# peach-xiao/EMRT

Measured on AMD Instinct MI355X. Metric: training tiles/sec at 256x256, higher is better.
Workload: dtype bf16; 1 GPU; EMRT ResNet50, Potsdam 256x256, 6 classes, batch 8 per GPU, fwd+bwd+SGD step (BASELINE configs[1]), bf16; global_batch=8, parallelism=dp1, hipgraph=True

## Files before the change

### emrt_amd/csrc/common.hpp

```cpp
#pragma once
#include <hip/hip_runtime.h>
#include <stdint.h>
#include <stdio.h>
#include <string.h>
#include "../../include/emrt_hip.h"

#define EMRT_F32 0
#define EMRT_BF16 1
#define EMRT_F16 2

namespace emrt {

extern thread_local char g_err[512];
inline int fail(const char* fn, const char* msg) {
  snprintf(g_err, sizeof(g_err), "%s: %s", fn, msg);
  return -1;
}
inline int check_launch(const char* fn) {
  hipError_t e = hipGetLastError();
  if (e != hipSuccess) {
    snprintf(g_err, sizeof(g_err), "%s: launch failed: %s", fn, hipGetErrorString(e));
    return -2;
  }
  return 0;
}
#define EMRT_REQUIRE(cond, msg) \
  do {                          \
    if (!(cond)) return emrt::fail(__func__, msg); \
  } while (0)

struct Tuning {
  int conv_tile;
  int wgrad_split;
  int thin_cblk;
  int thin_blocks;
  int thin_ch;
  int no_thin_bwd;
  int igemm64_nst;
  int wgrad_nst;
  int pair_max;
  int msda_fwd_global;
  int msda_bwd_global;
  int msda_lds_min_pairs;
  int msda_bwd_dref_lds;
  int msda_band_halo;
  int msda_scatter_qsplit;
  int msda_scatter_cuts;
  int msda_fwd_chunks;
  int msda_fwd_threads;
  int msda_fwd_probe;
  int bn_block_kb;
  int bn_slice_c;
  int bn_operand_blocks;
  int ln_bwd_rows;
  int ln_bwd_max_blocks;
  int ln_bwd_threads;
  int ln_atomic;
  int gn_group_blocks;
  int gn_stat_rows;
  int gn_bwd_stat_rows;
  int gn_apply_rows;
  int igemm8p_probe;
  int igemm8p_cmajor;
  int igemm8p_min_blocks;
  int wgrad8p_min_steps;
  int wgrad8p_slab;
  int wgrad8p_xcd;
  int wgrad8p_force;
  int no_ksplit128;
  int wgrad_no_overwrite;
  int no_s2_dgrad;
  int wgroup_blocks;
  int wgroup_min_steps;
  int wgroup_max;
  int wgroup8;
  int wgroup8_blocks;
  int wgroup8_min_work;
  int msda_scatter_merge;
  int msda_scatter_mfma;
  int msda_mf_bands;
  int sgd_nt;
  int mha_bwd_split;
  int mha_valu;
  int no_bna;
  int memcpy_kernel;
  int xk;
};
extern Tuning g_tune;

struct Scratch {
  void* ptr; size_t bytes; void* stream;
  unsigned* tick;
  float* xk_part;
};
constexpr size_t SCRATCH_TICK_BYTES = 65536;
constexpr int SCRATCH_TICKS = (int)(SCRATCH_TICK_BYTES / 4);
constexpr size_t SCRATCH_XK_BYTES = 8u << 20;
extern Scratch g_scratch;

struct bf16_t {
  unsigned short v;
};
struct f16_t {
  unsigned short v;
};

__device__ __forceinline__ float to_f32(float x) { return x; }
__device__ __forceinline__ float to_f32(bf16_t x) { return __uint_as_float(((uint32_t)x.v) << 16); }
__device__ __forceinline__ float to_f32(f16_t x) { return (float)__builtin_bit_cast(_Float16, x.v); }
__device__ __forceinline__ float bf16_bits_to_f32(uint32_t lo16) { return __uint_as_float(lo16 << 16); }
__device__ __forceinline__ float f16_bits_to_f32(uint32_t lo16) { return (float)__builtin_bit_cast(_Float16, (unsigned short)lo16); }

template <class T>
__device__ __forceinline__ T from_f32(float f);
template <>
__device__ __forceinline__ float from_f32<float>(float f) {
  return f;
}
template <>
__device__ __forceinline__ bf16_t from_f32<bf16_t>(float f) {
  __bf16 b = (__bf16)f;
  bf16_t r;
  r.v = __builtin_bit_cast(unsigned short, b);
  return r;
}
template <>
__device__ __forceinline__ f16_t from_f32<f16_t>(float f) {
  f16_t r;
  r.v = __builtin_bit_cast(unsigned short, (_Float16)f);
  return r;
}
typedef __attribute__((ext_vector_type(2))) _Float16 emrt_half2_t;
typedef __attribute__((ext_vector_type(2))) float emrt_float2_t;
__device__ __forceinline__ uint32_t pack_f16x2(float lo, float hi) {
  emrt_half2_t h = __builtin_convertvector((emrt_float2_t){lo, hi}, emrt_half2_t);
  return __builtin_bit_cast(uint32_t, h);
}
__device__ __forceinline__ void unpack_f16x2(uint32_t w, float& lo, float& hi) {
  const emrt_half2_t h = __builtin_bit_cast(emrt_half2_t, w);
  lo = (float)h.x;
  hi = (float)h.y;
}
__device__ __forceinline__ uint32_t pack_bf16x2(float lo, float hi) {
  return (uint32_t)from_f32<bf16_t>(lo).v | ((uint32_t)from_f32<bf16_t>(hi).v << 16);
}

template <class T>
struct Vec4;
template <>
struct Vec4<float> {
  __device__ static __forceinline__ void load(const float* p, float (&o)[4]) {
    float4 v = *reinterpret_cast<const float4*>(p);
    o[0] = v.x; o[1] = v.y; o[2] = v.z; o[3] = v.w;
  }
  __device__ static __forceinline__ void store(float* p, const float (&o)[4]) {
    *reinterpret_cast<float4*>(p) = make_float4(o[0], o[1], o[2], o[3]);
  }
// ... 230 lines not shown
```

### emrt_amd/csrc/conv.hip

```cpp
#include "common.hpp"
#include "bn_operand.hpp"
#include <stdlib.h>
#include <type_traits>

using namespace emrt;

typedef __attribute__((ext_vector_type(8))) __bf16 bf16x8_t;
typedef __attribute__((ext_vector_type(4))) short short4_t;
typedef __attribute__((ext_vector_type(16))) float f32x16_t;

struct ConvArgs {
  const void* in = nullptr;
  const void* w = nullptr;
  void* out = nullptr;
  const float* bias = nullptr;
  const float* scale = nullptr;
  const void* res = nullptr;
  int N = 0, H = 0, W = 0, C = 0, ldin = 0;
  long long in_bs = 0;
  int OH = 0, OW = 0, OC = 0, ldout = 0;
  long long out_bs = 0;
  int ldres = 0;
  long long res_bs = 0;
  int KH = 0, KW = 0, stride = 0, pad = 0;
  int dil = 1;
  int relu = 0, out_f32 = 0;
  int cmajor = 0;
  double* stats = nullptr;
  const void* mask_y = nullptr;
  float mask_scale = 1.f;
  const void* stat_x = nullptr;
  int ldsx = 0;
  long long sx_bs = 0;
  int ldy = 0;
  long long y_bs = 0;
  int xk_S = 0;
  float* xk_part = nullptr;
  unsigned* xk_tick = nullptr;
  const unsigned long long* drop_seed = nullptr;
  unsigned drop_salt = 0;
  float drop_p = 0.f;
  BnOperand bna = {};
  void* a_out = nullptr;
};

template <class T>
__device__ __forceinline__ void mma_chunk(f32x16_t& acc, const uint4& a, const uint4& b);
template <>
__device__ __forceinline__ void mma_chunk<bf16_t>(f32x16_t& acc, const uint4& a, const uint4& b) {
  acc = __builtin_amdgcn_mfma_f32_32x32x16_bf16(__builtin_bit_cast(bf16x8_t, a), __builtin_bit_cast(bf16x8_t, b), acc, 0, 0, 0);
}
typedef __attribute__((ext_vector_type(8))) _Float16 f16x8_t;
template <>
__device__ __forceinline__ void mma_chunk<f16_t>(f32x16_t& acc, const uint4& a, const uint4& b) {
  acc = __builtin_amdgcn_mfma_f32_32x32x16_f16(__builtin_bit_cast(f16x8_t, a), __builtin_bit_cast(f16x8_t, b), acc, 0, 0, 0);
}
template <>
__device__ __forceinline__ void mma_chunk<float>(f32x16_t& acc, const uint4& a, const uint4& b) {
  acc = __builtin_amdgcn_mfma_f32_32x32x2f32(__uint_as_float(a.x), __uint_as_float(b.x), acc, 0, 0, 0);
  acc = __builtin_amdgcn_mfma_f32_32x32x2f32(__uint_as_float(a.y), __uint_as_float(b.y), acc, 0, 0, 0);
  acc = __builtin_amdgcn_mfma_f32_32x32x2f32(__uint_as_float(a.z), __uint_as_float(b.z), acc, 0, 0, 0);
  acc = __builtin_amdgcn_mfma_f32_32x32x2f32(__uint_as_float(a.w), __uint_as_float(b.w), acc, 0, 0, 0);
}

constexpr unsigned BUF_RANGE = 0x80000000u;
constexpr unsigned BUF_OOB = 0x80000000u;
typedef __attribute__((ext_vector_type(4))) unsigned int u32x4_t;
__device__ __forceinline__ uint4 buf_load16(__amdgpu_buffer_rsrc_t rs, unsigned off) {
  const u32x4_t v = __builtin_amdgcn_raw_buffer_load_b128(rs, (int)off, 0, 0);
  return make_uint4(v.x, v.y, v.z, v.w);
}
template <class T>
__device__ __forceinline__ uint32_t buf_load_elem(__amdgpu_buffer_rsrc_t rs, unsigned off);
template <>
__device__ __forceinline__ uint32_t buf_load_elem<bf16_t>(__amdgpu_buffer_rsrc_t rs, unsigned off) {
  return (uint32_t)(unsigned short)__builtin_amdgcn_raw_buffer_load_b16(rs, (int)off, 0, 0);
}
template <>
__device__ __forceinline__ uint32_t buf_load_elem<f16_t>(__amdgpu_buffer_rsrc_t rs, unsigned off) {
  return (uint32_t)(unsigned short)__builtin_amdgcn_raw_buffer_load_b16(rs, (int)off, 0, 0);
}
template <>
__device__ __forceinline__ uint32_t buf_load_elem<float>(__amdgpu_buffer_rsrc_t rs, unsigned off) {
  return (uint32_t)__builtin_amdgcn_raw_buffer_load_b32(rs, (int)off, 0, 0);
// ... 1281 lines not shown
  if (G > 1 && lds < (size_t)(G - 1) * 16 * 256 * 4) lds = (size_t)(G - 1) * 16 * 256 * 4;
  static bool attr_done = false;
  if (!attr_done) {
    if (hipFuncSetAttribute(reinterpret_cast<const void*>(igemm_bna_kernel<T, 2>), hipFuncAttributeMaxDynamicSharedMemorySize, 160 * 1024) != hipSuccess ||
        hipFuncSetAttribute(reinterpret_cast<const void*>(igemm_bna_kernel<T, 4>), hipFuncAttributeMaxDynamicSharedMemorySize, 160 * 1024) != hipSuccess)
      return fail("emrt_conv2d_bna", "cannot raise the dynamic LDS limit");
    attr_done = true;
  }
  if (G == 1) hipLaunchKernelGGL((igemm_bna_kernel<T, 1>), dim3((unsigned)nb), dim3(256), lds, st, a);
  else if (G == 2) hipLaunchKernelGGL((igemm_bna_kernel<T, 2>), dim3((unsigned)nb), dim3(512), lds, st, a);
  else hipLaunchKernelGGL((igemm_bna_kernel<T, 4>), dim3((unsigned)nb), dim3(1024), lds, st, a);
  return check_launch("emrt_conv2d_bna");
}

static ConvArgs bna_args(const void* in, const void* w_packed, void* out, const float* bias, const void* residual, int N, int H, int W, int C, int ldin,
                         long long in_bs, int OH, int OW, int OC, int ldout, long long out_bs, int ldres, long long res_bs, int KH, int KW, int stride, int pad,
                         int relu, int out_f32, double* bn_stats, int dilation, const double* sums, double count, float eps, float momentum, float* mean,
                         float* invstd, float* run_mean, float* run_var, const float* gamma, const float* beta, int in_relu, void* a_out) {
  ConvArgs a = conv_fwd_args(in, w_packed, out, bias, residual, N, H, W, C, ldin, in_bs, OH, OW, OC, ldout, out_bs, ldres, res_bs, KH, KW, stride, pad, dilation,
                             relu, out_f32, bn_stats, 0, nullptr);
  a.bna.sums = sums; a.bna.inv_count = count > 0.0 ? 1.0 / count : 0.0; a.bna.eps = eps; a.bna.momentum = momentum; a.bna.mean = mean; a.bna.invstd = invstd;
  a.bna.run_mean = run_mean; a.bna.run_var = run_var; a.bna.gamma = gamma; a.bna.beta = beta; a.bna.relu = in_relu;
  a.a_out = a_out;
  return a;
}

extern "C" int emrt_conv2d_bna_supported(const void* in, const void* w_packed, void* out, const float* bias, const void* residual, int N, int H, int W, int C,
                                         int ldin, long long in_bs, int OH, int OW, int OC, int ldout, long long out_bs, int ldres, long long res_bs, int KH,
                                         int KW, int stride, int pad, int relu, int out_f32, double* bn_stats, int dilation, const double* sums, double count,
                                         float eps, float momentum, float* mean, float* invstd, float* run_mean, float* run_var, const float* gamma,
                                         const float* beta, int in_relu, void* a_out, int dtype, void* stream) {
  if (!(dtype == EMRT_F32 || dtype == EMRT_BF16) || !in || !w_packed || !out || !sums || !mean || !invstd || !gamma || !beta || !a_out || count <= 0.0) return 0;
  if (N <= 0 || H <= 0 || W <= 0 || C <= 0 || OC <= 0 || dilation < 1 || g_tune.no_bna == 1) return 0;
  const long long esz = dtype == EMRT_F32 ? 4 : 2;
  if ((long long)N * H * W * C * esz >= (1ll << 31) || (long long)N * H * W + 512 >= (1ll << 31)) return 0;
  if (((long long)(N - 1) * in_bs + ((long long)H * W - 1) * ldin + C) * esz >= (1ll << 31) || (long long)OC * KH * KW * C * esz >= (1ll << 31)) return 0;
  const ConvArgs a = bna_args(in, w_packed, out, bias, residual, N, H, W, C, ldin, in_bs, OH, OW, OC, ldout, out_bs, ldres, res_bs, KH, KW, stride, pad, relu, out_f32,
                              bn_stats, dilation, sums, count, eps, momentum, mean, invstd, run_mean, run_var, gamma, beta, in_relu, a_out);
  hipStream_t st = (hipStream_t)stream;
  return with_train_dtype("emrt_conv2d_bna_supported", dtype, [&](auto t) { return bna_plan<decltype(t)>(a, st).kind != CONV_NONE ? 1 : 0; });
}

extern "C" int emrt_conv2d_bna(const void* in, const void* w_packed, void* out, const float* bias, const void* residual, int N, int H, int W, int C,
                               int ldin, long long in_bs, int OH, int OW, int OC, int ldout, long long out_bs, int ldres, long long res_bs, int KH,
                               int KW, int stride, int pad, int relu, int out_f32, double* bn_stats, int dilation, const double* sums, double count,
                               float eps, float momentum, float* mean, float* invstd, float* run_mean, float* run_var, const float* gamma,
                               const float* beta, int in_relu, void* a_out, int dtype, void* stream) {
  EMRT_REQUIRE_TRAIN_DTYPE(dtype);
  EMRT_REQUIRE(in && w_packed && out && sums && mean && invstd && gamma && beta && a_out, "null pointer");
  const ConvShape s = {N, H, W, C, OH, OW, OC, KH, KW, stride, pad, dilation};
  EMRT_CONV_CHECK(s, 0, 0, 0, 0, dtype, CK_DIMS);
  EMRT_REQUIRE(dilation >= 1 && count > 0.0, "bad dims");
  EMRT_REQUIRE((run_mean != nullptr) == (run_var != nullptr), "running statistics come in pairs");
  EMRT_REQUIRE(a_out != out && a_out != in, "a_out is a buffer of its own");
  EMRT_REQUIRE((long long)N * OH * OW + 512 < (1ll << 31), "more than 2^31 pixels (32-bit pixel arithmetic)");
  EMRT_CONV_CHECK(s, ldin, in_bs, 0, 0, dtype, CK_X | CK_W);
  EMRT_REQUIRE((long long)N * H * W * C * (dtype == EMRT_F32 ? 4 : 2) < (1ll << 31), "operand spans 2 GiB or more (32-bit buffer offsets)");
  const ConvArgs a = bna_args(in, w_packed, out, bias, residual, N, H, W, C, ldin, in_bs, OH, OW, OC, ldout, out_bs, ldres, res_bs, KH, KW, stride, pad, relu, out_f32,
                              bn_stats, dilation, sums, count, eps, momentum, mean, invstd, run_mean, run_var, gamma, beta, in_relu, a_out);
  hipStream_t st = (hipStream_t)stream;
  return with_train_dtype("emrt_conv2d_bna", dtype, [&](auto t) {
    using T = decltype(t);
    const ConvPlan plan = bna_plan<T>(a, st);
    if (plan.kind == CONV_NONE) return fail("emrt_conv2d_bna", "this layer has no operand-transform kernel (ask emrt_conv2d_bna_supported first)");
    return launch_bna<T>(a, st, plan);
  });
}

template <class T>
static bool wgrad_is_vec(const WgradArgs& a) {
  constexpr int EPC = 16 / (int)sizeof(T);
  return (a.C % EPC == 0) && (a.OC % EPC == 0) && (a.ldx % EPC == 0) && (a.lddy % EPC == 0) && (a.x_bs % EPC == 0) && (a.dy_bs % EPC == 0) &&
         (((uintptr_t)a.x) % 16 == 0) && (((uintptr_t)a.dy) % 16 == 0);
}

template <class T>
static void wgrad_plan(WgradArgs& a, int& tx, int& ty, int& S_out) {
  using Cfg = WgradCfg<T>;
  const int K = a.KH * a.KW * a.C;
  const long long M = (long long)a.N * a.OH * a.OW;
  tx = (K + 127) / 128;
  ty = (a.OC + 127) / 128;
  const long long mt_total = (M + Cfg::BKM - 1) / Cfg::BKM;
  const double atom_us = (double)tx * 128.0 * (double)ty * 128.0 * 4.0 / 1.3e6;
  long long S = 1;
  double best = 1e30;
  static const int cand[] = {1, 2, 4, 8, 16, 32, 64, 128};
  for (int ci = 0; ci < (int)(sizeof(cand) / sizeof(cand[0])); ++ci) {
    const long long sc = cand[ci];
    if (sc > mt_total) break;
    if (sc > 1 && (long long)tx * ty >= 256) break;
    const double per = (double)((mt_total + sc - 1) / sc);
    const double nblk = (double)tx * ty * sc;
    const double t = per * (nblk > 1024.0 ? nblk / 1024.0 : 1.0) + sc * atom_us;
    if (t < best) { best = t; S = sc; }
  }
  if (g_tune.wgrad_split > 0) S = g_tune.wgrad_split < mt_total ? g_tune.wgrad_split : mt_total;
  a.tiles_per_split = (int)((mt_total + S - 1) / S);
  S_out = (int)((mt_total + a.tiles_per_split - 1) / a.tiles_per_split);
}

#include "wgrad8p.hpp"

template <class T>
static int wgrad_dispatch(const WgradArgs& a0, hipStream_t st) {
  using Cfg = WgradCfg<T>;
  WgradArgs a = a0;
  if constexpr (std::is_same<T, bf16_t>::value) {
    int tk, toc, S8, per;
    if (wgrad8p_plan<T>(a, tk, toc, S8, per)) return launch_wgrad8p(a, tk, toc, S8, per, st);
  }
  const bool vec = wgrad_is_vec<T>(a);
  int tx, ty, S;
  wgrad_plan<T>(a, tx, ty, S);
  if (S > 1 || !vec || g_tune.wgrad_no_overwrite) a.overwrite = 0;
  constexpr int G = 1;
  const int gv = vec ? G : 1;
  const size_t lds = (size_t)gv * 2 * 2 * Cfg::BKM * Cfg::PITCH;
  static bool attr_done = false;
  if (!attr_done) {
    if (hipFuncSetAttribute(reinterpret_cast<const void*>(wgrad_kernel<T, true, G>), hipFuncAttributeMaxDynamicSharedMemorySize,
                            (int)((size_t)G * 4 * Cfg::BKM * Cfg::PITCH)) != hipSuccess ||
        hipFuncSetAttribute(reinterpret_cast<const void*>(wgrad_kernel<T, false, 1>), hipFuncAttributeMaxDynamicSharedMemorySize,
                            (int)((size_t)4 * Cfg::BKM * Cfg::PITCH)) != hipSuccess)
      return fail("emrt_conv2d_wgrad", "cannot raise the dynamic LDS limit");
    attr_done = true;
  }
  const int xcd = g_tune.wgrad8p_xcd;
  const unsigned grid1 = 8u * (unsigned)(((long long)tx * ty * S + 7) / 8);
  if (vec && g_tune.wgrad_nst == 3) {
    static bool attr3 = false;
    if (!attr3) { (void)hipFuncSetAttribute(reinterpret_cast<const void*>(wgrad_kernel<T, true, G, 3>), hipFuncAttributeMaxDynamicSharedMemorySize, (int)((size_t)G * 4 * Cfg::BKM * Cfg::PITCH)); attr3 = true; }
    hipLaunchKernelGGL((wgrad_kernel<T, true, G, 3>), dim3(grid1), dim3(256 * G), lds, st, a, tx, ty, S, xcd);
  } else if (vec) hipLaunchKernelGGL((wgrad_kernel<T, true, G>), dim3(grid1), dim3(256 * G), lds, st, a, tx, ty, S, xcd);
  else hipLaunchKernelGGL((wgrad_kernel<T, false, 1>), dim3(grid1), dim3(256), lds, st, a, tx, ty, S, xcd);
  return check_launch("emrt_conv2d_wgrad");
}

extern "C" int emrt_conv2d_wgrad(const void* x, const void* dy, float* dw,
                                 int N, int H, int W, int C, int ldx, long long x_bs,
                                 int OH, int OW, int OC, int lddy, long long dy_bs,
                                 int KH, int KW, int stride, int pad, float* dbias, int dilation, int dtype, void* stream) {
  EMRT_REQUIRE(x && dy && dw, "null pointer");
  const ConvShape s = {N, H, W, C, OH, OW, OC, KH, KW, stride, pad, dilation};
  EMRT_CONV_CHECK(s, ldx, x_bs, lddy, dy_bs, dtype, CK_DIMS);
  EMRT_REQUIRE(dilation >= 1, "bad dims");
  EMRT_CONV_CHECK(s, ldx, x_bs, lddy, dy_bs, dtype, CK_SIZE | CK_PIXELS);
  EMRT_REQUIRE_TRAIN_DTYPE(dtype);
  EMRT_CONV_CHECK(s, ldx, x_bs, lddy, dy_bs, dtype, CK_X | CK_Y | CK_X24);
  const WgradArgs a = wgrad_args(x, dy, dw, dbias, N, H, W, C, ldx, x_bs, OH, OW, OC, lddy, dy_bs, KH, KW, stride, pad, dilation, 0);
  hipStream_t st = (hipStream_t)stream;
  return with_train_dtype("emrt_conv2d_wgrad", dtype, [&](auto t) { return wgrad_dispatch<decltype(t)>(a, st); });
}

struct ThinBwdArgs {
  const void* x; const void* dy; const void* wd; void* dx; float* dw; float* dbias; double* stats; const void* mask_y;
  int HW, C, OC, ldx, lddy, lddx, ldy, accumulate, pix_per_block, cg_shift;
  float mask_scale;
  long long x_bs, dy_bs, dx_bs, y_bs, M;
  const float* bn_mean; const float* bn_invstd; const float* bn_gamma; const float* bn_beta;
};

template <class T, int CH>
struct VecN;
template <class T>
struct VecN<T, 4> : Vec4<T> {};
template <class T>
struct VecN<T, 8> : Vec8<T> {};

template <class T, int CH, int MASK, bool ACC, bool BNX = false>
__global__ __launch_bounds__(256, CH == 4 ? 4 : 2) void thin_bwd_kernel(ThinBwdArgs p) {
  constexpr int U = 2;
  using V = VecN<T, CH>;
  __shared__ float red[32 * 256];
  const T* x = (const T*)p.x;
  const T* dy = (const T*)p.dy;
  const T* wd = (const T*)p.wd;
  const T* ym = (const T*)p.mask_y;
  T* dx = (T*)p.dx;
// ... 519 lines not shown
    w = wgrad_args(b.x, b.dy, b.dw, b.dbias, b.N, b.H, b.W, b.C, b.ldx, b.x_bs, b.OH, b.OW, b.OC, b.lddy, b.dy_bs, b.KH, b.KW, b.stride, b.pad, 1, 0);
    const bool vec = conv_is_vec<T>(d) && wgrad_is_vec<T>(w) && d.OC > 32;
    groupable = groupable && vec;
    int tx = 1, ty = 1, S = 1;
    if (vec) wgrad_plan<T>(w, tx, ty, S);
    g.nd[i] = (int)conv_blocks(d, 64, 64);
    g.wtx[i] = tx; g.wty[i] = ty;
    g.first[i] = (int)total;
    total += g.nd[i] + (long long)tx * ty * S;
  }
  for (int i = n; i <= EMRT_MAX_GROUP; ++i) g.first[i] = (int)total;
  for (int i = n; i < EMRT_MAX_GROUP; ++i) { g.d[i] = g.d[0]; g.w[i] = g.w[0]; g.nd[i] = 0; g.wtx[i] = 1; g.wty[i] = 1; }
  if (!groupable || total > 4096) {
    for (int i = 0; i < n; ++i) {
      const int rc = conv_bwd_dispatch<T>(g.d[i], g.w[i], st);
      if (rc) return rc;
    }
    return 0;
  }
  auto kern = bwd_group_kernel<T>;
  const size_t lds_d = (size_t)2 * 128 * 144, lds_w = (size_t)4 * Cfg::BKM * Cfg::PITCH;
  const size_t lds = lds_d > lds_w ? lds_d : lds_w;
  static bool attr_done = false;
  if (!attr_done) {
    if (hipFuncSetAttribute(reinterpret_cast<const void*>(kern), hipFuncAttributeMaxDynamicSharedMemorySize, (int)lds) != hipSuccess)
      return fail("emrt_conv2d_bwd_group", "cannot raise the dynamic LDS limit");
    attr_done = true;
  }
  hipLaunchKernelGGL(kern, dim3((unsigned)total), dim3(256), lds, st, g);
  return check_launch("emrt_conv2d_bwd_group");
}

extern "C" int emrt_conv2d_bwd_group(const EmrtConvBwdDesc* descs, int n, int dtype, void* stream) {
  EMRT_REQUIRE(descs && n >= 1 && n <= EMRT_MAX_GROUP, "1..6 problems");
  EMRT_REQUIRE_TRAIN_DTYPE(dtype);
  for (int i = 0; i < n; ++i) {
    const EmrtConvBwdDesc& b = descs[i];
    EMRT_REQUIRE(b.x && b.dy && b.w_bwd_packed && b.dx, "null pointer");
    EMRT_REQUIRE((b.dw == nullptr) == (descs[0].dw == nullptr) && (b.dw || !b.dbias), "dw == NULL (data gradients only) must hold for every problem of the group, without dbias");
    const ConvShape s = {b.N, b.H, b.W, b.C, b.OH, b.OW, b.OC, b.KH, b.KW, b.stride, b.pad, 1};
    EMRT_CONV_CHECK(s, b.ldx, b.x_bs, b.lddy, b.dy_bs, dtype, CK_GROUPED | CK_DIMS | CK_SIZE | CK_PIXELS);
    EMRT_REQUIRE(b.lddx >= b.C && b.dx_bs >= 0, "bad dx strides");
    EMRT_CONV_CHECK(s, b.ldx, b.x_bs, b.lddy, b.dy_bs, dtype, CK_GROUPED | CK_X | CK_Y | CK_X24);
  }
  hipStream_t st = (hipStream_t)stream;
  return with_train_dtype("emrt_conv2d_bwd_group", dtype, [&](auto t) { return conv_bwd_group_dispatch<decltype(t)>(descs, n, st); });
}

template <class T>
static int conv_dgrad_multi_dispatch(const EmrtConvDgradDesc* descs, int n, hipStream_t st) {
  ConvGroupArgs g;
  for (int i = 0; i < n; ++i) {
    const EmrtConvDgradDesc& b = descs[i];
    g.p[i] = conv_dgrad_args(b.dy, b.w_bwd_packed, b.dx, b.lddx, b.dx_bs, b.accumulate, b.addend, b.ldadd, b.add_bs, b.N, b.H, b.W, b.C, b.OH, b.OW, b.OC, b.lddy,
                             b.dy_bs, b.KH, b.KW, b.stride, b.pad, b.dilation, g_tune.igemm8p_cmajor, b.bn_stats, b.mask_y, b.ldy, b.y_bs, b.mask_scale, b.stat_x,
                             b.ldsx, b.sx_bs);
  }
  if (n == 1) return conv_dispatch<T, 1>(g.p[0], st);
  return conv_group_launch<T, 1>(g, n, 2048, "emrt_conv2d_dgrad_multi", st);
}

extern "C" int emrt_conv2d_dgrad_multi(const EmrtConvDgradDesc* descs, int n, int dtype, void* stream) {
  EMRT_REQUIRE(descs && n >= 1 && n <= EMRT_MAX_GROUP, "1..6 problems");
  EMRT_REQUIRE_TRAIN_DTYPE(dtype);
  for (int i = 0; i < n; ++i) {
    const EmrtConvDgradDesc& b = descs[i];
    EMRT_REQUIRE(b.dy && b.w_bwd_packed && b.dx, "null pointer");
    const ConvShape s = {b.N, b.H, b.W, b.C, b.OH, b.OW, b.OC, b.KH, b.KW, b.stride, b.pad, b.dilation};
    EMRT_CONV_CHECK(s, 0, 0, b.lddy, b.dy_bs, dtype, CK_DIMS | CK_KERNEL | CK_SIZE | CK_PIXELS | CK_Y | CK_W | CK_Y24);
    EMRT_REQUIRE(b.lddx >= b.C && b.dx_bs >= 0, "bad dx strides");
    EMRT_REQUIRE(!(b.accumulate && b.addend), "accumulate adds into dx itself; addend is a different tensor");
    EMRT_REQUIRE(!b.stat_x || b.mask_y, "stat_x replaces the mask tensor in the second statistic: it needs mask_y");
    for (int j = 0; j < i; ++j) EMRT_REQUIRE(descs[j].dx != b.dx, "two problems of one launch must not write the same dx");
  }
  hipStream_t st = (hipStream_t)stream;
  return with_train_dtype("emrt_conv2d_dgrad_multi", dtype, [&](auto t) { return conv_dgrad_multi_dispatch<decltype(t)>(descs, n, st); });
}

#define EMRT_MAX_WGROUP 24
struct WgradGroupArgs {
  WgradArgs w[EMRT_MAX_WGROUP];
  int first[EMRT_MAX_WGROUP + 1];
  short wtx[EMRT_MAX_WGROUP], wty[EMRT_MAX_WGROUP];
  int n, xcd;
};

template <class T>
__global__ __launch_bounds__(256, 2) void wgrad_group_kernel(WgradGroupArgs g) {
  extern __shared__ __attribute__((aligned(16))) unsigned char smem_all[];
  const int nb = g.first[g.n];
  int w = (int)blockIdx.x;
  if (g.xcd) {
    const int k = w & 7, idx = w >> 3;
    const int w0 = (int)(((long long)k * nb) >> 3), w1 = (int)(((long long)(k + 1) * nb) >> 3);
    w = w0 + idx;
    if (w >= w1) return;
  } else if (w >= nb) return;
  int i = 0;
  for (int k = 1; k < g.n; ++k) i += w >= g.first[k] ? 1 : 0;
  i = __builtin_amdgcn_readfirstlane(i);
  const int local = w - g.first[i];
  const int tx = g.wtx[i], ty = g.wty[i];
  const int bz = __builtin_amdgcn_readfirstlane(local / (tx * ty)), t = __builtin_amdgcn_readfirstlane(local - bz * (tx * ty));
  const int by = __builtin_amdgcn_readfirstlane(t / tx);
  wgrad_body<T, true, 1>(g.w[i], __builtin_amdgcn_readfirstlane(t - by * tx), by, bz, smem_all);
}

static WgradArgs wgrad_args_from_desc(const EmrtWgradDesc& d) {
  return wgrad_args(d.x, d.dy, d.dw, d.dbias, d.N, d.H, d.W, d.C, d.ldx, d.x_bs, d.OH, d.OW, d.OC, d.lddy, d.dy_bs, d.KH, d.KW, d.stride, d.pad, d.dilation,
                    d.dw_is_zero ? 1 : 0);
}

template <class T>
static int wgrad_group_dispatch(const EmrtWgradDesc* descs, int n, hipStream_t st) {
  using Cfg = WgradCfg<T>;
  WgradArgs pend[EMRT_MAX_WGROUP];
  int npend = 0;
  auto flush = [&]() -> int {
    if (npend == 0) return 0;
    if (npend == 1) { const int rc = wgrad_dispatch<T>(pend[0], st); npend = 0; return rc; }
    int tx[EMRT_MAX_WGROUP], ty[EMRT_MAX_WGROUP], S1[EMRT_MAX_WGROUP];
    long long mt[EMRT_MAX_WGROUP], work = 0;
    for (int i = 0; i < npend; ++i) {
      WgradArgs tmp = pend[i];
      wgrad_plan<T>(tmp, tx[i], ty[i], S1[i]);
      mt[i] = ((long long)pend[i].N * pend[i].OH * pend[i].OW + Cfg::BKM - 1) / Cfg::BKM;
      work += (long long)tx[i] * ty[i] * mt[i];
    }
    int order[EMRT_MAX_WGROUP];
    long long tps[EMRT_MAX_WGROUP], Sl[EMRT_MAX_WGROUP];
    {
      long long Tt = (work + g_tune.wgroup_blocks - 1) / (g_tune.wgroup_blocks > 0 ? g_tune.wgroup_blocks : 1024);
      if (Tt < g_tune.wgroup_min_steps) Tt = g_tune.wgroup_min_steps;
      if (Tt < 1) Tt = 1;
      for (int i = 0; i < npend; ++i) {
        long long S = (mt[i] + Tt - 1) / Tt;
        Sl[i] = S > S1[i] ? S1[i] : (S < 1 ? 1 : S);
      }
    }
    for (int i = 0; i < npend; ++i) {
      tps[i] = (mt[i] + Sl[i] - 1) / Sl[i];
      order[i] = i;
    }
    for (int i = 1; i < npend; ++i)
      for (int j = i; j > 0 && tps[order[j]] > tps[order[j - 1]]; --j) { const int t_ = order[j]; order[j] = order[j - 1]; order[j - 1] = t_; }
    WgradGroupArgs g;
    long long total = 0;
    for (int q = 0; q < npend; ++q) {
      const int i = order[q];
      g.w[q] = pend[i];
      g.w[q].tiles_per_split = (int)tps[i];
      const long long S = (mt[i] + tps[i] - 1) / tps[i];
      if (S > 1 || g_tune.wgrad_no_overwrite) g.w[q].overwrite = 0;
      g.first[q] = (int)total;
      g.wtx[q] = (short)tx[i]; g.wty[q] = (short)ty[i];
      total += (long long)tx[i] * ty[i] * S;
    }
    for (int q = npend; q <= EMRT_MAX_WGROUP; ++q) g.first[q] = (int)total;
    for (int q = npend; q < EMRT_MAX_WGROUP; ++q) { g.w[q] = g.w[0]; g.wtx[q] = 1; g.wty[q] = 1; }
    g.n = npend; g.xcd = g_tune.wgrad8p_xcd;
    npend = 0;
    if (total >= (1ll << 30)) return fail("emrt_conv2d_wgrad_group", "too many blocks");
    auto kern = wgrad_group_kernel<T>;
    const size_t lds = (size_t)4 * Cfg::BKM * Cfg::PITCH;
    static bool attr_done = false;
    if (!attr_done) {
      if (hipFuncSetAttribute(reinterpret_cast<const void*>(kern), hipFuncAttributeMaxDynamicSharedMemorySize, (int)lds) != hipSuccess)
        return fail("emrt_conv2d_wgrad_group", "cannot raise the dynamic LDS limit");
      attr_done = true;
    }
    hipLaunchKernelGGL(kern, dim3(8u * (unsigned)((total + 7) / 8)), dim3(256), lds, st, g);
    return check_launch("emrt_conv2d_wgrad_group");
  };
  WgradArgs pend8[EMRT_MAX_WGROUP8];
  int npend8 = 0;
  auto flush8 = [&]() -> int {
    if (npend8 == 0) return 0;
    const int rc = launch_wgrad8p_group(pend8, npend8, st);
    npend8 = 0;
    return rc;
  };
  auto aliased = [&](int i) { for (int j = 0; j < n; ++j) if (j != i && descs[j].dw == descs[i].dw) return true; return false; };
  long long work8 = 0;
  if constexpr (std::is_same<T, bf16_t>::value) {
    for (int i = 0; i < n && g_tune.wgroup8 > 0; ++i) {
      const WgradArgs a = wgrad_args_from_desc(descs[i]);
      int tk, toc, S8, per, tiles8, steps8;
      if (wgrad_is_vec<T>(a) && !wgrad8p_plan<T>(a, tk, toc, S8, per) && wgrad8p_group_ok<T>(a, tiles8, steps8) && !aliased(i)) work8 += (long long)tiles8 * steps8;
    }
  }
  const bool use8 = g_tune.wgroup8 > 0 && work8 >= (g_tune.wgroup8_min_work > 0 ? g_tune.wgroup8_min_work : 1);
  for (int i = 0; i < n; ++i) {
    WgradArgs a = wgrad_args_from_desc(descs[i]);
    const bool alias = aliased(i);
    if (alias) a.overwrite = 0;
    bool alone = !wgrad_is_vec<T>(a) || a.KH * a.KW * a.C >= 32768 * 128 || a.OC >= 32768 * 128;
    if constexpr (std::is_same<T, bf16_t>::value) {
      int tk, toc, S8, per;
      if (wgrad8p_plan<T>(a, tk, toc, S8, per)) alone = true;
    }
    if (alone) {
      const int rc = wgrad_dispatch<T>(a, st);
      if (rc) return rc;
      continue;
    }
    if constexpr (std::is_same<T, bf16_t>::value) {
      int tiles8, steps8;
      if (use8 && !alias && wgrad8p_group_ok<T>(a, tiles8, steps8)) {
        pend8[npend8++] = a;
        if (npend8 == EMRT_MAX_WGROUP8) {
          const int rc = flush8();
          if (rc) return rc;
        }
        continue;
      }
    }
    pend[npend++] = a;
    if (npend == EMRT_MAX_WGROUP || (g_tune.wgroup_max > 0 && npend >= g_tune.wgroup_max)) {
      const int rc = flush();
      if (rc) return rc;
    }
  }
  {
    const int rc = flush8();
    if (rc) return rc;
  }
  return flush();
}

extern "C" int emrt_conv2d_wgrad_group(const EmrtWgradDesc* descs, int n, int dtype, void* stream) {
  EMRT_REQUIRE(descs && n >= 1, "no problems");
  EMRT_REQUIRE_TRAIN_DTYPE(dtype);
  for (int i = 0; i < n; ++i) {
    const EmrtWgradDesc& d = descs[i];
    EMRT_REQUIRE(d.x && d.dy && d.dw, "null pointer");
    const ConvShape s = {d.N, d.H, d.W, d.C, d.OH, d.OW, d.OC, d.KH, d.KW, d.stride, d.pad, d.dilation};
    EMRT_CONV_CHECK(s, d.ldx, d.x_bs, d.lddy, d.dy_bs, dtype, CK_DIMS);
    EMRT_REQUIRE(d.dilation >= 1, "bad dims");
    EMRT_CONV_CHECK(s, d.ldx, d.x_bs, d.lddy, d.dy_bs, dtype, CK_KERNEL | CK_SIZE | CK_PIXELS | CK_X | CK_Y | CK_X24);
  }
  hipStream_t st = (hipStream_t)stream;
  return with_train_dtype("emrt_conv2d_wgrad_group", dtype, [&](auto t) { return wgrad_group_dispatch<decltype(t)>(descs, n, st); });
}
```

### emrt_amd/csrc/elementwise.hip

```cpp
#include "common.hpp"
#include <stdlib.h>

using namespace emrt;

thread_local char emrt::g_err[512] = {0};

extern "C" const char* emrt_last_error(void) { return emrt::g_err; }
extern "C" int emrt_abi_version(void) { return 9; }

namespace {
struct TuneEntry { const char* name; int emrt::Tuning::*field; int def; };
const TuneEntry kTune[] = {
    {"conv_tile", &emrt::Tuning::conv_tile, 0},         {"wgrad_split", &emrt::Tuning::wgrad_split, 0},
    {"thin_cblk", &emrt::Tuning::thin_cblk, 64},        {"thin_blocks", &emrt::Tuning::thin_blocks, 128},
    {"thin_ch", &emrt::Tuning::thin_ch, 8},             {"no_thin_bwd", &emrt::Tuning::no_thin_bwd, 0},
    {"pair_max", &emrt::Tuning::pair_max, 768},         {"msda_fwd_global", &emrt::Tuning::msda_fwd_global, 0},
    {"bn_block_kb", &emrt::Tuning::bn_block_kb, 0},     {"ln_atomic", &emrt::Tuning::ln_atomic, 1},
    {"bn_slice_c", &emrt::Tuning::bn_slice_c, 0},
    {"msda_fwd_chunks", &emrt::Tuning::msda_fwd_chunks, 0}, {"msda_fwd_threads", &emrt::Tuning::msda_fwd_threads, 1024},
    {"msda_fwd_probe", &emrt::Tuning::msda_fwd_probe, 0}, {"wgrad_nst", &emrt::Tuning::wgrad_nst, 2},
    {"igemm64_nst", &emrt::Tuning::igemm64_nst, 3}, {"msda_bwd_global", &emrt::Tuning::msda_bwd_global, 0},
    {"msda_lds_min_pairs", &emrt::Tuning::msda_lds_min_pairs, 2048}, {"msda_bwd_dref_lds", &emrt::Tuning::msda_bwd_dref_lds, 1},
    {"gn_group_blocks", &emrt::Tuning::gn_group_blocks, 0}, {"gn_stat_rows", &emrt::Tuning::gn_stat_rows, 32},
    {"gn_bwd_stat_rows", &emrt::Tuning::gn_bwd_stat_rows, 32}, {"gn_apply_rows", &emrt::Tuning::gn_apply_rows, 8},
    {"msda_scatter_cuts", &emrt::Tuning::msda_scatter_cuts, 0}, {"msda_scatter_qsplit", &emrt::Tuning::msda_scatter_qsplit, 0}, {"msda_band_halo", &emrt::Tuning::msda_band_halo, 0},
    {"igemm8p_probe", &emrt::Tuning::igemm8p_probe, 0}, {"igemm8p_min_blocks", &emrt::Tuning::igemm8p_min_blocks, 160}, {"igemm8p_cmajor", &emrt::Tuning::igemm8p_cmajor, 0},
    {"wgrad8p_min_steps", &emrt::Tuning::wgrad8p_min_steps, 8}, {"wgrad8p_slab", &emrt::Tuning::wgrad8p_slab, 1}, {"wgrad8p_force", &emrt::Tuning::wgrad8p_force, 0}, {"wgrad8p_xcd", &emrt::Tuning::wgrad8p_xcd, 1},
    {"wgrad_no_overwrite", &emrt::Tuning::wgrad_no_overwrite, 0}, {"no_ksplit128", &emrt::Tuning::no_ksplit128, 0}, {"ln_bwd_rows", &emrt::Tuning::ln_bwd_rows, 0}, {"ln_bwd_max_blocks", &emrt::Tuning::ln_bwd_max_blocks, 0}, {"bn_operand_blocks", &emrt::Tuning::bn_operand_blocks, 0}, {"no_s2_dgrad", &emrt::Tuning::no_s2_dgrad, 0}, {"wgroup_blocks", &emrt::Tuning::wgroup_blocks, 1024}, {"wgroup_min_steps", &emrt::Tuning::wgroup_min_steps, 32}, {"wgroup_max", &emrt::Tuning::wgroup_max, 0},
    {"no_bna", &emrt::Tuning::no_bna, 0}, {"memcpy_kernel", &emrt::Tuning::memcpy_kernel, 0}, {"xk", &emrt::Tuning::xk, 0}, {"mha_valu", &emrt::Tuning::mha_valu, 0}, {"mha_bwd_split", &emrt::Tuning::mha_bwd_split, 1}, {"msda_scatter_merge", &emrt::Tuning::msda_scatter_merge, 0},
    {"wgroup8", &emrt::Tuning::wgroup8, 0}, {"wgroup8_blocks", &emrt::Tuning::wgroup8_blocks, 0}, {"wgroup8_min_work", &emrt::Tuning::wgroup8_min_work, 6000},
    {"msda_scatter_mfma", &emrt::Tuning::msda_scatter_mfma, 1}, {"sgd_nt", &emrt::Tuning::sgd_nt, 1}, {"ln_bwd_threads", &emrt::Tuning::ln_bwd_threads, 512}, {"msda_mf_bands", &emrt::Tuning::msda_mf_bands, 0},
};
emrt::Tuning tuning_from_env() {
  emrt::Tuning t;
  for (const TuneEntry& e : kTune) {
    char env[64] = "EMRT_";
    size_t n = strlen(env);
    for (const char* c = e.name; *c && n + 1 < sizeof(env); ++c) env[n++] = (char)((*c >= 'a' && *c <= 'z') ? *c - 32 : *c);
    env[n] = 0;
    const char* v = (strcmp(e.name, "msda_fwd_probe") == 0 || strcmp(e.name, "igemm8p_probe") == 0) ? nullptr : getenv(env);
    t.*(e.field) = v ? atoi(v) : e.def;
  }
  return t;
}
}
emrt::Tuning emrt::g_tune = tuning_from_env();
emrt::Scratch emrt::g_scratch = {nullptr, 0, nullptr, nullptr, nullptr};

extern "C" int emrt_set_scratch(void* ptr, size_t bytes, void* stream) {
  EMRT_REQUIRE((ptr != nullptr) == (bytes > 0) && ((uintptr_t)ptr) % 256 == 0, "scratch must be 256-byte aligned device memory (or nullptr, 0)");
  if (ptr && ptr == emrt::g_scratch.ptr && emrt::g_scratch.tick && bytes == emrt::g_scratch.bytes + emrt::SCRATCH_TICK_BYTES + emrt::SCRATCH_XK_BYTES) {
    emrt::g_scratch.stream = stream;
    return 0;
  }
  emrt::g_scratch.ptr = ptr;
  emrt::g_scratch.bytes = bytes;
  emrt::g_scratch.stream = stream;
  emrt::g_scratch.tick = nullptr;
  emrt::g_scratch.xk_part = nullptr;
  if (ptr && bytes >= (16u << 20) + emrt::SCRATCH_XK_BYTES + emrt::SCRATCH_TICK_BYTES && bytes % 256 == 0) {
    emrt::g_scratch.bytes = bytes - emrt::SCRATCH_TICK_BYTES - emrt::SCRATCH_XK_BYTES;
    emrt::g_scratch.xk_part = reinterpret_cast<float*>(static_cast<char*>(ptr) + emrt::g_scratch.bytes);
    emrt::g_scratch.tick = reinterpret_cast<unsigned*>(static_cast<char*>(ptr) + emrt::g_scratch.bytes + emrt::SCRATCH_XK_BYTES);
    if (hipMemsetAsync(emrt::g_scratch.tick, 0, emrt::SCRATCH_TICK_BYTES, (hipStream_t)stream) != hipSuccess) {
      emrt::g_scratch.tick = nullptr;
      return emrt::fail("emrt_set_scratch", "cannot zero the arrival counters");
    }
  }
  return 0;
}

extern "C" int emrt_set_tuning(const char* name, int value) {
  EMRT_REQUIRE(name, "null name");
  for (const TuneEntry& e : kTune)
    if (strcmp(e.name, name) == 0) { emrt::g_tune.*(e.field) = value; return 0; }
  return emrt::fail("emrt_set_tuning", "unknown knob");
}
extern "C" int emrt_get_tuning(const char* name, int* value) {
  EMRT_REQUIRE(name && value, "null pointer");
  for (const TuneEntry& e : kTune)
    if (strcmp(e.name, name) == 0) { *value = emrt::g_tune.*(e.field); return 0; }
  return emrt::fail("emrt_get_tuning", "unknown knob");
}

static inline int ew_grid(long long total) {
  long long g = (total + 255) / 256;
  if (g > 8192) g = 8192;
  if (g < 1) g = 1;
  return (int)g;
}

template <class T>
__global__ __launch_bounds__(256) void add_kernel(const T* __restrict__ a, const T* __restrict__ b, T* __restrict__ out, long long n4,
                                                  long long period4) {
  for (long long i = (long long)blockIdx.x * blockDim.x + threadIdx.x; i < n4; i += (long long)gridDim.x * blockDim.x) {
    float x[4], y[4];
    Vec4<T>::load(a + i * 4, x);
    Vec4<T>::load(b + ((n4 | period4) <= 0xffffffffll ? (long long)((unsigned)i % (unsigned)period4) : i % period4) * 4, y);
#pragma unroll
    for (int e = 0; e < 4; ++e) x[e] += y[e];
    Vec4<T>::store(out + i * 4, x);
  }
}

template <class T>
__global__ __launch_bounds__(256) void add_f32row_kernel(const T* __restrict__ a, const float* __restrict__ b, T* __restrict__ out,
                                                         long long n4, long long period4) {
  for (long long i = (long long)blockIdx.x * blockDim.x + threadIdx.x; i < n4; i += (long long)gridDim.x * blockDim.x) {
    float x[4];
    Vec4<T>::load(a + i * 4, x);
    const float4 y = reinterpret_cast<const float4*>(b)[(n4 | period4) <= 0xffffffffll ? (long long)((unsigned)i % (unsigned)period4) : i % period4];
// ... 371 lines not shown
```

Baseline: 1041 tiles/s.

## Plan grouped wgrad slicing and XCD partition with a cost-model simulator

Moves the grouped weight-gradient planner into a header. The planner now splits blocks across the eight XCDs by modelled cost instead of by block count. It also searches several slice-depth targets and a keep-fresh option, scores each with a simple list-scheduling simulation that includes an atomic-bandwidth floor, and memoizes the choice per problem signature. The goal is to balance per-XCD work and avoid needless split-K atomics. The cost constants are hand-fitted and may mispredict, and the grid now depends on the longest XCD range.

After: 1049 tiles/s (median of 6 runs). Within noise of the previous version (+0.7%).

```diff
diff --git a/emrt_amd/csrc/common.hpp b/emrt_amd/csrc/common.hpp
--- a/emrt_amd/csrc/common.hpp
+++ b/emrt_amd/csrc/common.hpp
@@ -73,6 +73,8 @@
   int wgroup_blocks;
   int wgroup_min_steps;
   int wgroup_max;
+  int wgroup_xcd_cost;
+  int wgroup_tsim;
   int wgroup8;
   int wgroup8_blocks;
   int wgroup8_min_work;
diff --git a/emrt_amd/csrc/conv.hip b/emrt_amd/csrc/conv.hip
--- a/emrt_amd/csrc/conv.hip
+++ b/emrt_amd/csrc/conv.hip
@@ -1,5 +1,6 @@
 #include "common.hpp"
 #include "bn_operand.hpp"
+#include "wgrad_group_plan.hpp"
 #include <stdlib.h>
 #include <type_traits>
 
@@ -1447,19 +1448,7 @@
   tx = (K + 127) / 128;
   ty = (a.OC + 127) / 128;
   const long long mt_total = (M + Cfg::BKM - 1) / Cfg::BKM;
-  const double atom_us = (double)tx * 128.0 * (double)ty * 128.0 * 4.0 / 1.3e6;
-  long long S = 1;
-  double best = 1e30;
-  static const int cand[] = {1, 2, 4, 8, 16, 32, 64, 128};
-  for (int ci = 0; ci < (int)(sizeof(cand) / sizeof(cand[0])); ++ci) {
-    const long long sc = cand[ci];
-    if (sc > mt_total) break;
-    if (sc > 1 && (long long)tx * ty >= 256) break;
-    const double per = (double)((mt_total + sc - 1) / sc);
-    const double nblk = (double)tx * ty * sc;
-    const double t = per * (nblk > 1024.0 ? nblk / 1024.0 : 1.0) + sc * atom_us;
-    if (t < best) { best = t; S = sc; }
-  }
+  long long S = emrt_wgplan::alone_slices(tx, ty, mt_total);
   if (g_tune.wgrad_split > 0) S = g_tune.wgrad_split < mt_total ? g_tune.wgrad_split : mt_total;
   a.tiles_per_split = (int)((mt_total + S - 1) / S);
   S_out = (int)((mt_total + a.tiles_per_split - 1) / a.tiles_per_split);
@@ -2145,8 +2134,10 @@
   WgradArgs w[EMRT_MAX_WGROUP];
   int first[EMRT_MAX_WGROUP + 1];
   short wtx[EMRT_MAX_WGROUP], wty[EMRT_MAX_WGROUP];
+  int xfirst[9];
   int n, xcd;
 };
+static_assert(sizeof(WgradGroupArgs) <= 4096, "WgradGroupArgs travels as a kernel argument: 4 KiB at most");
 
 template <class T>
 __global__ __launch_bounds__(256, 2) void wgrad_group_kernel(WgradGroupArgs g) {
@@ -2155,9 +2146,8 @@
   int w = (int)blockIdx.x;
   if (g.xcd) {
     const int k = w & 7, idx = w >> 3;
-    const int w0 = (int)(((long long)k * nb) >> 3), w1 = (int)(((long long)(k + 1) * nb) >> 3);
-    w = w0 + idx;
-    if (w >= w1) return;
+    w = g.xfirst[k] + idx;
+    if (w >= g.xfirst[k + 1]) return;
   } else if (w >= nb) return;
   int i = 0;
   for (int k = 1; k < g.n; ++k) i += w >= g.first[k] ? 1 : 0;
@@ -2182,45 +2172,36 @@
   auto flush = [&]() -> int {
     if (npend == 0) return 0;
     if (npend == 1) { const int rc = wgrad_dispatch<T>(pend[0], st); npend = 0; return rc; }
-    int tx[EMRT_MAX_WGROUP], ty[EMRT_MAX_WGROUP], S1[EMRT_MAX_WGROUP];
-    long long mt[EMRT_MAX_WGROUP], work = 0;
+    int tx[EMRT_MAX_WGROUP], ty[EMRT_MAX_WGROUP];
+    emrt_wgplan::Problem prob[EMRT_MAX_WGROUP];
     for (int i = 0; i < npend; ++i) {
       WgradArgs tmp = pend[i];
-      wgrad_plan<T>(tmp, tx[i], ty[i], S1[i]);
-      mt[i] = ((long long)pend[i].N * pend[i].OH * pend[i].OW + Cfg::BKM - 1) / Cfg::BKM;
-      work += (long long)tx[i] * ty[i] * mt[i];
-    }
-    int order[EMRT_MAX_WGROUP];
-    long long tps[EMRT_MAX_WGROUP], Sl[EMRT_MAX_WGROUP];
-    {
-      long long Tt = (work + g_tune.wgroup_blocks - 1) / (g_tune.wgroup_blocks > 0 ? g_tune.wgroup_blocks : 1024);
-      if (Tt < g_tune.wgroup_min_steps) Tt = g_tune.wgroup_min_steps;
-      if (Tt < 1) Tt = 1;
-      for (int i = 0; i < npend; ++i) {
-        long long S = (mt[i] + Tt - 1) / Tt;
-        Sl[i] = S > S1[i] ? S1[i] : (S < 1 ? 1 : S);
-      }
-    }
-    for (int i = 0; i < npend; ++i) {
-      tps[i] = (mt[i] + Sl[i] - 1) / Sl[i];
-      order[i] = i;
-    }
-    for (int i = 1; i < npend; ++i)
-      for (int j = i; j > 0 && tps[order[j]] > tps[order[j - 1]]; --j) { const int t_ = order[j]; order[j] = order[j - 1]; order[j - 1] = t_; }
+      int S1;
+      wgrad_plan<T>(tmp, tx[i], ty[i], S1);
+      prob[i].tiles = tx[i] * ty[i];
+      prob[i].mt = ((long long)pend[i].N * pend[i].OH * pend[i].OW + Cfg::BKM - 1) / Cfg::BKM;
+      prob[i].cap = S1;
+      prob[i].fresh = (pend[i].overwrite && !g_tune.wgrad_no_overwrite) ? 1 : 0;
+    }
+    emrt_wgplan::Knobs kn;
+    kn.blocks = g_tune.wgroup_blocks; kn.min_steps = g_tune.wgroup_min_steps; kn.cost_cut = g_tune.wgroup_xcd_cost ? 1 : 0; kn.simulate = g_tune.wgroup_tsim ? 1 : 0;
+    static emrt_wgplan::Memo memo;
+    const emrt_wgplan::Plan plan = emrt_wgplan::plan_batch(prob, npend, kn, &memo);
+    const long long total = plan.total;
     WgradGroupArgs g;
-    long long total = 0;
     for (int q = 0; q < npend; ++q) {
-      const int i = order[q];
+      const int i = plan.order[q];
       g.w[q] = pend[i];
-      g.w[q].tiles_per_split = (int)tps[i];
-      const long long S = (mt[i] + tps[i] - 1) / tps[i];
-      if (S > 1 || g_tune.wgrad_no_overwrite) g.w[q].overwrite = 0;
-      g.first[q] = (int)total;
+      g.w[q].tiles_per_split = (int)plan.tps[q];
+      g.w[q].overwrite = plan.store[q];
+      g.first[q] = plan.first[q];
       g.wtx[q] = (short)tx[i]; g.wty[q] = (short)ty[i];
-      total += (long long)tx[i] * ty[i] * S;
-    }
-    for (int q = npend; q <= EMRT_MAX_WGROUP; ++q) g.first[q] = (int)total;
+    }
+    for (int q = npend; q <= EMRT_MAX_WGROUP; ++q) g.first[q] = plan.first[npend];
     for (int q = npend; q < EMRT_MAX_WGROUP; ++q) { g.w[q] = g.w[0]; g.wtx[q] = 1; g.wty[q] = 1; }
+    int longest = 0;
+    for (int k = 0; k <= 8; ++k) g.xfirst[k] = plan.xfirst[k];
+    for (int k = 0; k < 8; ++k) longest = g.xfirst[k + 1] - g.xfirst[k] > longest ? g.xfirst[k + 1] - g.xfirst[k] : longest;
     g.n = npend; g.xcd = g_tune.wgrad8p_xcd;
     npend = 0;
     if (total >= (1ll << 30)) return fail("emrt_conv2d_wgrad_group", "too many blocks");
@@ -2232,7 +2213,8 @@
         return fail("emrt_conv2d_wgrad_group", "cannot raise the dynamic LDS limit");
       attr_done = true;
     }
-    hipLaunchKernelGGL(kern, dim3(8u * (unsigned)((total + 7) / 8)), dim3(256), lds, st, g);
+    const unsigned grid = g.xcd ? 8u * (unsigned)longest : (unsigned)total;
+    hipLaunchKernelGGL(kern, dim3(grid), dim3(256), lds, st, g);
     return check_launch("emrt_conv2d_wgrad_group");
   };
   WgradArgs pend8[EMRT_MAX_WGROUP8];
diff --git a/emrt_amd/csrc/elementwise.hip b/emrt_amd/csrc/elementwise.hip
--- a/emrt_amd/csrc/elementwise.hip
+++ b/emrt_amd/csrc/elementwise.hip
@@ -27,6 +27,7 @@
     {"igemm8p_probe", &emrt::Tuning::igemm8p_probe, 0}, {"igemm8p_min_blocks", &emrt::Tuning::igemm8p_min_blocks, 160}, {"igemm8p_cmajor", &emrt::Tuning::igemm8p_cmajor, 0},
     {"wgrad8p_min_steps", &emrt::Tuning::wgrad8p_min_steps, 8}, {"wgrad8p_slab", &emrt::Tuning::wgrad8p_slab, 1}, {"wgrad8p_force", &emrt::Tuning::wgrad8p_force, 0}, {"wgrad8p_xcd", &emrt::Tuning::wgrad8p_xcd, 1},
     {"wgrad_no_overwrite", &emrt::Tuning::wgrad_no_overwrite, 0}, {"no_ksplit128", &emrt::Tuning::no_ksplit128, 0}, {"ln_bwd_rows", &emrt::Tuning::ln_bwd_rows, 0}, {"ln_bwd_max_blocks", &emrt::Tuning::ln_bwd_max_blocks, 0}, {"bn_operand_blocks", &emrt::Tuning::bn_operand_blocks, 0}, {"no_s2_dgrad", &emrt::Tuning::no_s2_dgrad, 0}, {"wgroup_blocks", &emrt::Tuning::wgroup_blocks, 1024}, {"wgroup_min_steps", &emrt::Tuning::wgroup_min_steps, 32}, {"wgroup_max", &emrt::Tuning::wgroup_max, 0},
+    {"wgroup_xcd_cost", &emrt::Tuning::wgroup_xcd_cost, 1}, {"wgroup_tsim", &emrt::Tuning::wgroup_tsim, 1},
     {"no_bna", &emrt::Tuning::no_bna, 0}, {"memcpy_kernel", &emrt::Tuning::memcpy_kernel, 0}, {"xk", &emrt::Tuning::xk, 0}, {"mha_valu", &emrt::Tuning::mha_valu, 0}, {"mha_bwd_split", &emrt::Tuning::mha_bwd_split, 1}, {"msda_scatter_merge", &emrt::Tuning::msda_scatter_merge, 0},
     {"wgroup8", &emrt::Tuning::wgroup8, 0}, {"wgroup8_blocks", &emrt::Tuning::wgroup8_blocks, 0}, {"wgroup8_min_work", &emrt::Tuning::wgroup8_min_work, 6000},
     {"msda_scatter_mfma", &emrt::Tuning::msda_scatter_mfma, 1}, {"sgd_nt", &emrt::Tuning::sgd_nt, 1}, {"ln_bwd_threads", &emrt::Tuning::ln_bwd_threads, 512}, {"msda_mf_bands", &emrt::Tuning::msda_mf_bands, 0},
diff --git a/emrt_amd/csrc/wgrad_group_plan.hpp b/emrt_amd/csrc/wgrad_group_plan.hpp
--- /dev/null
+++ b/emrt_amd/csrc/wgrad_group_plan.hpp
@@ -0,0 +1,244 @@
+#pragma once
+#include <cstdint>
+
+namespace emrt_wgplan {
+
+constexpr int kMaxProblems = 24;
+constexpr int kXcds = 8;
+constexpr int kSlots = 64;
+constexpr int kMaxSimItems = 1 << 15;
+
+constexpr double kC1 = 1.107;
+constexpr double kC0Store = 10.2;
+constexpr double kC0Atomic = 16.6;
+constexpr double kAtomicBytesPerUs = 1.3e6;
+
+struct Problem {
+  int tiles;
+  long long mt;
+  int cap;
+  int fresh;
+};
+
+struct Knobs {
+  int blocks = 1024;
+  int min_steps = 32;
+  int cost_cut = 1;
+  int simulate = 1;
+};
+
+struct Plan {
+  int n = 0;
+  int order[kMaxProblems];
+  long long tps[kMaxProblems];
+  int slices[kMaxProblems];
+  int store[kMaxProblems];
+  int first[kMaxProblems + 1];
+  int xfirst[kXcds + 1];
+  long long T = 0;
+  int keep_fresh = 0;
+  int cut = 0;
+  double makespan = -1.0;
+  long long total = 0;
+};
+
+inline long long alone_slices(int tx, int ty, long long mt_total) {
+  const double atom_us = (double)tx * 128.0 * (double)ty * 128.0 * 4.0 / 1.3e6;
+  long long S = 1;
+  double best = 1e30;
+  static const int cand[] = {1, 2, 4, 8, 16, 32, 64, 128};
+  for (int ci = 0; ci < (int)(sizeof(cand) / sizeof(cand[0])); ++ci) {
+    const long long sc = cand[ci];
+    if (sc > mt_total) break;
+    if (sc > 1 && (long long)tx * ty >= 256) break;
+    const double per = (double)((mt_total + sc - 1) / sc);
+    const double nblk = (double)tx * ty * sc;
+    const double t = per * (nblk > 1024.0 ? nblk / 1024.0 : 1.0) + sc * atom_us;
+    if (t < best) { best = t; S = sc; }
+  }
+  return S;
+}
+
+inline double item_cost(const Plan& p, int q) { return (p.store[q] ? kC0Store : kC0Atomic) + kC1 * (double)p.tps[q]; }
+
+inline long long rule_T(const Problem* pr, int n, const Knobs& kn) {
+  long long work = 0;
+  for (int i = 0; i < n; ++i) work += (long long)pr[i].tiles * pr[i].mt;
+  const long long blocks = kn.blocks > 0 ? kn.blocks : 1024;
+  long long T = (work + kn.blocks - 1) / blocks;
+  if (T < kn.min_steps) T = kn.min_steps;
+  return T < 1 ? 1 : T;
+}
+
+inline void cut_slices(const Problem* pr, int n, long long T, int keep_fresh, Plan& p) {
+  long long tps[kMaxProblems];
+  int sl[kMaxProblems];
+  p.n = n; p.T = T; p.keep_fresh = keep_fresh;
+  for (int i = 0; i < n; ++i) {
+    long long S = (pr[i].mt + T - 1) / T;
+    S = S > pr[i].cap ? pr[i].cap : (S < 1 ? 1 : S);
+    if (keep_fresh && pr[i].fresh) S = 1;
+    tps[i] = (pr[i].mt + S - 1) / S;
+    if (tps[i] < 1) tps[i] = 1;
+    sl[i] = (int)((pr[i].mt + tps[i] - 1) / tps[i]);
+    if (sl[i] < 1) sl[i] = 1;
+    p.order[i] = i;
+  }
+  for (int i = 1; i < n; ++i)
+    for (int j = i; j > 0 && tps[p.order[j]] > tps[p.order[j - 1]]; --j) { const int t_ = p.order[j]; p.order[j] = p.order[j - 1]; p.order[j - 1] = t_; }
+  long long total = 0;
+  for (int q = 0; q < n; ++q) {
+    const int i = p.order[q];
+    p.tps[q] = tps[i]; p.slices[q] = sl[i];
+    p.store[q] = (pr[i].fresh && sl[i] == 1) ? 1 : 0;
+    p.first[q] = (int)(total < INT32_MAX ? total : INT32_MAX);
+    total += (long long)pr[i].tiles * sl[i];
+  }
+  p.first[n] = (int)(total < INT32_MAX ? total : INT32_MAX);
+  p.total = total;
+}
+
+inline void cut_by_count(Plan& p) {
+  for (int k = 0; k <= kXcds; ++k) p.xfirst[k] = (int)(((long long)k * p.total) >> 3);
+  p.cut = 0;
+}
+
+inline void cut_by_cost(const Problem* pr, Plan& p) {
+  const int n = p.n;
+  double cum[kMaxProblems + 1], longest = 0.0;
+  cum[0] = 0.0;
+  for (int q = 0; q < n; ++q) {
+    const double len = item_cost(p, q);
+    cum[q + 1] = cum[q] + len * (double)(p.first[q + 1] - p.first[q]);
+    if (p.first[q + 1] > p.first[q] && len > longest) longest = len;
+  }
+  p.xfirst[0] = 0; p.xfirst[kXcds] = p.first[n];
+  for (int k = 1; k < kXcds; ++k) {
+    const double want = cum[n] * (double)k / (double)kXcds;
+    int q = 0;
+    while (q + 1 < n && cum[q + 1] <= want) ++q;
+    const double len = item_cost(p, q);
+    long long at = p.first[q] + (long long)((want - cum[q]) / len + 0.5);
+    if (at > p.first[q + 1]) at = p.first[q + 1];
+    const int tiles = pr[p.order[q]].tiles;
+    const long long local = at - p.first[q], lo = local / tiles * tiles, hi = lo + tiles;
+    const long long snap = p.first[q] + ((local - lo <= hi - local) ? lo : hi);
+    if (snap != at && (snap - at == 1 || at - snap == 1) && snap <= p.first[q + 1]) {
+      const double dev = cum[q] + len * (double)(snap - p.first[q]) - want;
+      if ((dev < 0 ? -dev : dev) <= 0.5 * longest) at = snap;
+    }
+    if (at < p.xfirst[k - 1]) at = p.xfirst[k - 1];
+    p.xfirst[k] = (int)at;
+  }
+  p.cut = 1;
+}
+
+inline double range_cost(const Plan& p, int k) {
+  double c = 0.0;
+  for (int q = 0; q < p.n; ++q) {
+    const int a = p.xfirst[k] > p.first[q] ? p.xfirst[k] : p.first[q], b = p.xfirst[k + 1] < p.first[q + 1] ? p.xfirst[k + 1] : p.first[q + 1];
+    if (b > a) c += item_cost(p, q) * (double)(b - a);
+  }
+  return c;
+}
+
+inline double simulate(const Problem* pr, const Plan& p) {
+  if (p.total > kMaxSimItems) return -1.0;
+  double makespan = 0.0, atomic_bytes = 0.0;
+  for (int q = 0; q < p.n; ++q)
+    if (!p.store[q]) atomic_bytes += (double)pr[p.order[q]].tiles * (double)p.slices[q] * 65536.0;
+  for (int k = 0; k < kXcds; ++k) {
+    double fin[kSlots];
+    for (int c = 0; c < kSlots; ++c) fin[c] = 0.0;
+    int q = 0;
+    for (int w = p.xfirst[k]; w < p.xfirst[k + 1]; ++w) {
+      while (q + 1 < p.n && w >= p.first[q + 1]) ++q;
+      int cmin = 0;
+      for (int c = 1; c < kSlots; ++c) cmin = fin[c] < fin[cmin] ? c : cmin;
+      fin[cmin] += item_cost(p, q);
+    }
+    for (int c = 0; c < kSlots; ++c) makespan = fin[c] > makespan ? fin[c] : makespan;
+  }
+  const double floor_us = atomic_bytes / kAtomicBytesPerUs;
+  return makespan > floor_us ? makespan : floor_us;
+}
+
+inline Plan plan_parent(const Problem* pr, int n, const Knobs& kn, bool want_makespan) {
+  Plan p;
+  cut_slices(pr, n, rule_T(pr, n, kn), 0, p);
+  cut_by_count(p);
+  if (want_makespan) p.makespan = simulate(pr, p);
+  return p;
+}
+
+struct Memo {
+  static constexpr int kEntries = 32;
+  unsigned long long key[kEntries];
+  long long T[kEntries];
+  int keep_fresh[kEntries], cut[kEntries];
+  double makespan[kEntries];
+  int used = 0;
+};
+
+inline unsigned long long signature(const Problem* pr, int n, const Knobs& kn) {
+  unsigned long long key = 1469598103934665603ull;
+  auto mix = [&](unsigned long long v) { key = (key ^ v) * 1099511628211ull; };
+  mix((unsigned long long)n); mix((unsigned long long)(unsigned)kn.blocks); mix((unsigned long long)(unsigned)kn.min_steps);
+  mix((unsigned long long)(kn.cost_cut * 2 + kn.simulate));
+  for (int i = 0; i < n; ++i) { mix((unsigned long long)pr[i].mt); mix((unsigned long long)(unsigned)pr[i].tiles); mix((unsigned long long)(unsigned)(pr[i].cap * 2 + pr[i].fresh)); }
+  return key;
+}
+
+inline Plan plan_batch(const Problem* pr, int n, const Knobs& kn, Memo* memo) {
+  Plan p;
+  const bool sim_T = kn.simulate != 0 && kn.blocks == 1024;
+  const long long T0 = rule_T(pr, n, kn);
+  auto build = [&](long long T, int keep_fresh, int cut) {
+    Plan c;
+    cut_slices(pr, n, T, keep_fresh, c);
+    if (cut) cut_by_cost(pr, c); else cut_by_count(c);
+    return c;
+  };
+  if (!sim_T && !kn.cost_cut) return build(T0, 0, 0);
+  const unsigned long long key = signature(pr, n, kn);
+  if (memo)
+    for (int m = 0; m < (memo->used < Memo::kEntries ? memo->used : Memo::kEntries); ++m)
+      if (memo->key[m] == key) {
+        p = build(memo->T[m], memo->keep_fresh[m], memo->cut[m]);
+        p.makespan = memo->makespan[m];
+        return p;
+      }
+  auto modelled = [&](long long T, int keep_fresh, int cut) {
+    Plan c = build(T, keep_fresh, cut);
+    c.makespan = simulate(pr, c);
+    return c;
+  };
+  p = modelled(T0, 0, kn.cost_cut);
+  if (sim_T && p.makespan >= 0.0) {
+    long long work = 0, longest = 1;
+    for (int i = 0; i < n; ++i) { work += (long long)pr[i].tiles * pr[i].mt; longest = pr[i].mt > longest ? pr[i].mt : longest; }
+    static const int aim[] = {256, 384, 512, 640, 768, 896, 1152, 1280, 1536, 2048, 3072};
+    Plan best = p;
+    for (int keep = 0; keep < 2; ++keep)
+      for (int ci = -1; ci < (int)(sizeof(aim) / sizeof(aim[0])); ++ci) {
+        long long T = ci < 0 ? longest : (work + aim[ci] - 1) / aim[ci];
+        if (T < kn.min_steps) T = kn.min_steps;
+        if (T < 1) T = 1;
+        if (T == T0 && !keep) continue;
+        const Plan c = modelled(T, keep, kn.cost_cut);
+        if (c.makespan >= 0.0 && c.makespan < best.makespan) best = c;
+      }
+    if (best.makespan < 0.98 * p.makespan) p = best;
+  }
+  if (kn.cost_cut && p.makespan >= 0.0) {
+    const Plan e = modelled(T0, 0, 0);
+    if (e.makespan < p.makespan) p = e;
+  }
+  if (memo) {
+    const int m = memo->used++ % Memo::kEntries;
+    memo->key[m] = key; memo->T[m] = p.T; memo->keep_fresh[m] = p.keep_fresh; memo->cut[m] = p.cut; memo->makespan[m] = p.makespan;
+  }
+  return p;
+}
+
+}
```
